# CodexploreRepo/deepfm

Hardware: AMD Instinct MI355X
Metric: train samples/sec DeepFM Criteo-shape bs4096 (higher is better)
Workload: dtype f32

## Files before the change

### deepfm_amd/_lib.py

```python

from __future__ import annotations

import ctypes as C
import os
from typing import Optional

_HERE = os.path.dirname(os.path.abspath(__file__))
LIB_PATH = os.environ.get("DFM_LIB_PATH") or os.path.join(_HERE, "lib", "libdeepfm_hip.so")

ABI_VERSION = 8

MAX_FIELDS = 64
MAX_RANKS = 64
ROWPLAN_CHUNK = 4096
SPARSE, DENSE, SEQUENCE = 0, 1, 2
COMBINER = {"mean": 0, "sum": 1, "max": 2}

c_float_p = C.c_void_p
c_int_p = C.c_void_p


class Field(C.Structure):
    _fields_ = [("kind", C.c_int32), ("dim", C.c_int32), ("vocab", C.c_int32), ("max_len", C.c_int32),
                ("combiner", C.c_int32), ("flat_offset", C.c_int32), ("stride2", C.c_int32),
# ... 98 lines not shown
    "dfm_bn_relu_dropout_backward": (_I, [_P, _P, _P, _P, _P, _L, _I, _F, _P, _I, _P, _P, _P, _P, _P]),
    "dfm_bce_workspace_bytes": (_SZ, [_L]),
    "dfm_bce_with_logits": (_I, [_P, _P, _L, _P, _P, _P, _P]),
    "dfm_gemm_workspace_bytes": (_SZ, [_I, _I, _I]),
    "dfm_gemm_f32": (_I, [_P, _L, _I, _P, _L, _I, _P, _L, _I, _I, _I, _P, _I, _P, _P]),
    "dfm_weight_grad_workspace_bytes": (_SZ, [_L, _I, _I]),
    "dfm_weight_grad_f32": (_I, [_P, _L, _P, _L, _L, _I, _I, _P, _L, _P, _I, _P, _P]),
    "dfm_attention_core_supported": (_I, [_I, _I, _I]),
    "dfm_attention_core_forward": (_I, [_P, _L, _I, _I, _I, _P, _P]),
    "dfm_attention_core_backward": (_I, [_P, _P, _L, _I, _I, _I, _P, _P]),
    "dfm_attention_qkv_core_supported": (_I, [_I, _I, _I, _I]),
    "dfm_attention_qkv_core_forward": (_I, [_P, _P, _P, _L, _I, _I, _I, _I, _P, _P]),
    "dfm_attention_qkv_core_backward": (_I, [_P, _P, _P, _P, _L, _I, _I, _I, _I, _P, _P]),
    "dfm_attention_block_supported": (_I, [_I, _I, _I, _I]),
    "dfm_attention_block_forward": (_I, [_P, _P, _P, _P, _P, _P, _P, _F, _L, _I, _I, _I, _I, _P, _P, _P, _P, _L, _P, _L,
                                         _P]),
    "dfm_attention_block_backward": (_I, [_P, _P, _P, _P, _P, _I, _L, _I, _I, _I, _I, _P, _P, _P, _L, _P, _P, _P]),
    "dfm_layernorm_workspace_bytes": (_SZ, [_L, _I]),
    "dfm_layernorm_forward": (_I, [_P, _P, _L, _I, _P, _P, _F, _P, _P, _L, _L, _P]),
    "dfm_layernorm_backward": (_I, [_P, _P, _P, _P, _L, _I, _P, _P, _P, _P, _P, _L, _L, _P]),
    "dfm_linear_bn_workspace_bytes": (_SZ, [_L, _I]),
    "dfm_linear_bn_forward": (_I, [_P, _L, _P, _P, _L, _I, _I, _P, _P, _P]),
    "dfm_bn_relu_dropout_apply": (_I, [_P, _L, _I, _P, _P, _P, _P, _P, _P, _P, _F, _F, _F, _P, _I, _P, _P]),
    "dfm_bn_bwd_workspace_bytes": (_SZ, [_L, _I]),
    "dfm_bn_backward_apply": (_I, [C.POINTER(BnBwd), _L, _I, C.POINTER(HeadTail), _P, _P]),
    "dfm_linear1_supported": (_I, [_I]),
    "dfm_linear1_forward": (_I, [_P, _L, _I, _P, _P, _P, _P]),
    "dfm_linear1_backward_splits": (_I, [_L]),
    "dfm_linear1_backward": (_I, [_P, _P, _L, _I, _P, _P, _P, _P]),
    "dfm_head_bce": (_I, [_P, _L, _I, _P, _P, _P, _P, _P, _P, _P, C.POINTER(BnBwd), _P]),
    "dfm_head_bn_bce": (_I, [_P, _P, _P, _P, _P, _F, _F, _L, _I, _P, _P, _P, _P, _P, _P, _P, C.POINTER(BnBwd), _P]),
    "dfm_linear_backward_workspace_bytes": (_SZ, [_L, _I, _I]),
    "dfm_linear_backward": (_I, [_P, _L, _I, _P, _I, _P, _P, C.POINTER(BnBwd), C.POINTER(FmBwd), _I, _P, _P]),
    "dfm_linear_backward_finish": (_I, [C.POINTER(SlabRef), _I, _P]),
    "dfm_linear_backward_splits": (_I, [_L, _I, _I]),
    "dfm_step_embedding_backward": (_I, [_P, _I, C.POINTER(_P), C.POINTER(FieldGrad), C.POINTER(C.c_int32), _I, _I, _I,
                                         _L, _P, _P, _P, _P, _P, _P, _P, _P, _I, _P, _L, _P]),
    "dfm_step_prepare_num_partials": (_L, [_I, _I, _I, _L]),
    "dfm_step_match_bytes": (_SZ, [_I, _I]),
    "dfm_step_prepare": (_I, [C.POINTER(Table), _I, _I, _I, _P, _P, _P, _P, _P, _F, _F, _P, _P, _L, _L,
                              C.POINTER(SlabRef), _I, _P, _I, _L, _P, _L, _P, _P]),
    "dfm_step_apply": (_I, [C.POINTER(Table), _I, _I, _I, _P, _P, _P, _P, _P, _P, _F, _F, _F, _F, _P, _P, _P, _P, _P,
                            _L, _I, _P]),
    "dfm_step_apply_plan": (_I, [C.POINTER(Table), _I, _I, _I, _P, _P, _P, _P, _P, _P, _F, _F, _F, _F, _P, _P, _P, _P, _P,
                                 _L, _I, _P, _L, _P, _I, _L, _P, _P, _P, _P, _P, _P]),
    "dfm_step_apply_plan_update": (_I, [_P, _P, C.POINTER(Table), _I, _I, _I, _P, _P, _P, _P, _P, _P, _F, _F, _F, _F, _P,
                                        _P, _P, _P, _P, _L, _I, _P, _L, _P, _I, _L, _P, _P, _P, _P, _P]),
    "dfm_step_apply_opt": (_I, [C.POINTER(Table), _I, _I, _I, _P, _P, _P, _P, _P, _P, C.POINTER(Optim), _P, _P, _P, _P,
                                _P, _L, _I, _P]),
    "dfm_step_apply_plan_opt": (_I, [C.POINTER(Table), _I, _I, _I, _P, _P, _P, _P, _P, _P, C.POINTER(Optim), _P, _P, _P,
                                     _P, _P, _L, _I, _P, _L, _P, _I, _L, _P, _P, _P, _P, _P, _P]),
    "dfm_step_apply_plan_opt_update": (_I, [_P, _P, C.POINTER(Table), _I, _I, _I, _P, _P, _P, _P, _P, _P,
                                            C.POINTER(Optim), _P, _P, _P, _P, _P, _L, _I, _P, _L, _P, _I, _L, _P, _P, _P,
                                            _P, _P]),
    "dfm_weight_grad_partial_blocks": (_I, [_L]),
    "dfm_weight_grad_partials_f32": (_I, [_P, _L, _P, _L, _L, _I, _I, _P, _P]),
    "dfm_weight_grad_partials_pair_f32": (_I, [_P, _L, _P, _L, _I, _I, _P, _P, _L, _P, _L, _I, _I, _P, _L, _P]),
    "dfm_layernorm_partial_blocks": (_I, [_L]),
    "dfm_partials_finish": (_I, [C.POINTER(PartialJob), _I, _P]),
    "dfm_tower_set_mode": (_I, [_I]),
    "dfm_tower_get_mode": (_I, []),
    "dfm_planes_bytes": (_SZ, [_L, _L]),
    "dfm_tower_x6_supported": (_I, [_L, _I, _I]),
    "dfm_split_planes": (_I, [C.POINTER(SplitJob), _I, _P]),
    "dfm_linear_bn_forward_x6": (_I, [_P, _L, _P, _P, _P, _L, _I, _I, _P, _P, _P]),
    "dfm_bn_relu_dropout_apply_planes": (_I, [_P, _L, _I, _P, _P, _P, _P, _P, _P, _P, _F, _F, _F, _P, _I, _P, _P, _P,
# ... 70 lines not shown
```

### deepfm_amd/csrc/gemm_core.h

```cpp
#pragma once

#include <type_traits>

#include "common.h"

namespace dfm {
namespace gemm {

typedef float f32x16 __attribute__((ext_vector_type(16)));

constexpr int BM = 64, BN = 64, BK = 32;
constexpr int LDS_STRIDE = BK + 1;
constexpr int kThreads = 512;

struct Smem {
  float a[2][BM * LDS_STRIDE];
  float b[2][BN * LDS_STRIDE];
};

struct TilePos {
  int tile, khalf;
  int wm, wn;
  int r, hf;
  __device__ __forceinline__ TilePos() {
// ... 52 lines not shown
__device__ __forceinline__ void store_slice(float* __restrict__ lds, const float4& vin, bool okv) {
  const int p = threadIdx.x;
  const float4 v = (!MASK || okv) ? vin : make_float4(0.f, 0.f, 0.f, 0.f);
  if (KC) {
    const int row = p >> 3, kq = (p & 7) * 4;
    float* d = lds + row * LDS_STRIDE + kq;
    d[0] = v.x; d[1] = v.y; d[2] = v.z; d[3] = v.w;
  } else {
    const int kk = p >> 4, rq = (p & 15) * 4;
    float* d = lds + rq * LDS_STRIDE + kk;
    d[0] = v.x; d[LDS_STRIDE] = v.y; d[2 * LDS_STRIDE] = v.z; d[3 * LDS_STRIDE] = v.w;
  }
}

template <bool KC, bool MASK, int J>
__device__ __forceinline__ void store_piece(float* __restrict__ lds, const float4& vin, bool okv) {
  const int p = threadIdx.x;
  const float e = J == 0 ? vin.x : (J == 1 ? vin.y : (J == 2 ? vin.z : vin.w));
  const float v = (!MASK || okv) ? e : 0.f;
  if (KC) lds[(p >> 3) * LDS_STRIDE + (p & 7) * 4 + J] = v;
  else lds[((p & 15) * 4 + J) * LDS_STRIDE + (p >> 4)] = v;
}

#ifndef GEMM_INTERLEAVE
#define GEMM_INTERLEAVE 1
#endif
#ifndef GEMM_INTERLEAVE_TAIL
#define GEMM_INTERLEAVE_TAIL 0
#endif
#ifndef GEMM_ABLATE
#define GEMM_ABLATE 0
#endif

constexpr int kPrefetch = 4;
constexpr int kFrag = BK / 4;

__device__ __forceinline__ void read_frags(const Smem& sm, int buf, const TilePos& pos, float (&fa)[kFrag],
                                           float (&fb)[kFrag]) {
  const float* pa = sm.a[buf] + (pos.wm + pos.r) * LDS_STRIDE + pos.hf + pos.khalf * (BK / 2);
  const float* pb = sm.b[buf] + (pos.wn + pos.r) * LDS_STRIDE + pos.hf + pos.khalf * (BK / 2);
#pragma unroll
  for (int i = 0; i < kFrag; ++i) { fa[i] = pa[2 * i]; fb[i] = pb[2 * i]; }
}

template <bool A_KC, bool B_KC, bool A_FAST, bool B_FAST, int J, bool CHECK>
__device__ __forceinline__ void pipe_step(const float* __restrict__ A, int64_t lda, const float* __restrict__ B,
                                          int64_t ldb, int M, int N, int m0, int n0, int kc, int ke, Smem& sm,
                                          const TilePos& pos, const SteadyPtr<A_KC>& spa, const SteadyPtr<B_KC>& spb,
                                          float4 (&va)[kPrefetch], float4 (&vb)[kPrefetch], bool (&oka)[kPrefetch],
                                          bool (&okb)[kPrefetch], float (&fa)[kFrag], float (&fb)[kFrag], f32x16& acc) {
  constexpr int b1 = (J + 1) & 1, b2 = J & 1, slot = (J + 2) % kPrefetch;
  constexpr bool kBareA = !CHECK && A_FAST, kBareB = !CHECK && B_FAST;
  if (CHECK && kc >= ke) return;
  float na[kFrag], nb[kFrag];
  if constexpr (GEMM_INTERLEAVE && (!CHECK || GEMM_INTERLEAVE_TAIL)) {
    const float* pa = sm.a[b1] + (pos.wm + pos.r) * LDS_STRIDE + pos.hf + pos.khalf * (BK / 2);
    const float* pb = sm.b[b1] + (pos.wn + pos.r) * LDS_STRIDE + pos.hf + pos.khalf * (BK / 2);
    static_assert(kFrag == 8, "the gap schedule below is written for 8 MFMAs per slice");
#define DFM_GAP(I, STORE)                                                                   \
    if (!(GEMM_ABLATE & 1)) acc = __builtin_amdgcn_mfma_f32_32x32x2f32(fa[I], fb[I], acc, 0, 0, 0); \
    else acc[I] += fa[I] + fb[I];                                                            \
    if (!(GEMM_ABLATE & 8)) { na[I] = pa[2 * (I)]; nb[I] = pb[2 * (I)]; } else { na[I] = fa[I]; nb[I] = fb[I]; } \
    if (!(GEMM_ABLATE & 4)) { STORE; }                                                      \
    __builtin_amdgcn_sched_barrier(0);
    __builtin_amdgcn_sched_barrier(0);
    DFM_GAP(0, (store_piece<A_KC, !kBareA, 0>(sm.a[b2], va[slot], oka[slot])))
    DFM_GAP(1, (store_piece<A_KC, !kBareA, 1>(sm.a[b2], va[slot], oka[slot])))
    DFM_GAP(2, (store_piece<A_KC, !kBareA, 2>(sm.a[b2], va[slot], oka[slot])))
    DFM_GAP(3, (store_piece<A_KC, !kBareA, 3>(sm.a[b2], va[slot], oka[slot])))
    DFM_GAP(4, (store_piece<B_KC, !kBareB, 0>(sm.b[b2], vb[slot], okb[slot])))
    DFM_GAP(5, (store_piece<B_KC, !kBareB, 1>(sm.b[b2], vb[slot], okb[slot])))
    DFM_GAP(6, (store_piece<B_KC, !kBareB, 2>(sm.b[b2], vb[slot], okb[slot])))
    DFM_GAP(7, (store_piece<B_KC, !kBareB, 3>(sm.b[b2], vb[slot], okb[slot])))
#undef DFM_GAP
    if (!(GEMM_ABLATE & 2)) {
    if (kBareA) { va[slot] = spa.load(kc + (kPrefetch + 2) * BK); oka[slot] = true; }
    else load_slice<A_KC, A_FAST>(A, lda, m0, M, kc + (kPrefetch + 2) * BK, ke, va[slot], oka[slot]);
    if (kBareB) { vb[slot] = spb.load(kc + (kPrefetch + 2) * BK); okb[slot] = true; }
    else load_slice<B_KC, B_FAST>(B, ldb, n0, N, kc + (kPrefetch + 2) * BK, ke, vb[slot], okb[slot]);
    }
    __builtin_amdgcn_sched_barrier(0);
  } else {
#pragma unroll
  for (int i = 0; i < kFrag; ++i) na[i] = nb[i] = 0.f;
  if (!CHECK || kc + BK < ke) read_frags(sm, b1, pos, na, nb);
  if (!CHECK || kc + 2 * BK < ke) {
    store_slice<A_KC, !kBareA>(sm.a[b2], va[slot], oka[slot]);
    store_slice<B_KC, !kBareB>(sm.b[b2], vb[slot], okb[slot]);
  }
  if (!CHECK || kc + (kPrefetch + 2) * BK < ke) {
    if (kBareA) { va[slot] = spa.load(kc + (kPrefetch + 2) * BK); oka[slot] = true; }
    else load_slice<A_KC, A_FAST>(A, lda, m0, M, kc + (kPrefetch + 2) * BK, ke, va[slot], oka[slot]);
    if (kBareB) { vb[slot] = spb.load(kc + (kPrefetch + 2) * BK); okb[slot] = true; }
    else load_slice<B_KC, B_FAST>(B, ldb, n0, N, kc + (kPrefetch + 2) * BK, ke, vb[slot], okb[slot]);
  }
  __builtin_amdgcn_sched_barrier(0);
#pragma unroll
  for (int i = 0; i < kFrag; ++i) acc = __builtin_amdgcn_mfma_f32_32x32x2f32(fa[i], fb[i], acc, 0, 0, 0);
  __builtin_amdgcn_sched_barrier(0);
  }
  if (!(GEMM_ABLATE & 16) || CHECK) __syncthreads();
#pragma unroll
  for (int i = 0; i < kFrag; ++i) { fa[i] = na[i]; fb[i] = nb[i]; }
}

template <bool A_KC, bool B_KC, bool A_FAST, bool B_FAST>
__device__ __forceinline__ void mainloop(const float* __restrict__ A, int64_t lda, const float* __restrict__ B,
                                         int64_t ldb, int M, int N, int m0, int n0, int kb, int ke, Smem& sm,
                                         const TilePos& pos, f32x16& acc) {
  static_assert(kPrefetch == 4, "the slot schedule below is written out for 4 slices in flight");
  const int lane = lane_id();
  float4 va[kPrefetch], vb[kPrefetch];
  bool oka[kPrefetch], okb[kPrefetch];
#pragma unroll
  for (int j = 0; j < kPrefetch; ++j) {
    oka[j] = okb[j] = false;
    va[j] = vb[j] = make_float4(0.f, 0.f, 0.f, 0.f);
    if (kb + j * BK < ke) {
      load_slice<A_KC, A_FAST>(A, lda, m0, M, kb + j * BK, ke, va[j], oka[j]);
      load_slice<B_KC, B_FAST>(B, ldb, n0, N, kb + j * BK, ke, vb[j], okb[j]);
    }
  }
  store_slice<A_KC>(sm.a[0], va[0], oka[0]);
  store_slice<B_KC>(sm.b[0], vb[0], okb[0]);
  store_slice<A_KC>(sm.a[1], va[1], oka[1]);
  store_slice<B_KC>(sm.b[1], vb[1], okb[1]);
#pragma unroll
  for (int j = 0; j < 2; ++j) {
    if (kb + (kPrefetch + j) * BK < ke) {
      load_slice<A_KC, A_FAST>(A, lda, m0, M, kb + (kPrefetch + j) * BK, ke, va[j], oka[j]);
      load_slice<B_KC, B_FAST>(B, ldb, n0, N, kb + (kPrefetch + j) * BK, ke, vb[j], okb[j]);
    }
  }
  __syncthreads();
  float fa[kFrag], fb[kFrag];
  read_frags(sm, 0, pos, fa, fb);
  __syncthreads();
  const SteadyPtr<A_KC> spa(A, lda, m0, M);
  const SteadyPtr<B_KC> spb(B, ldb, n0, N);
#define DFM_PIPE(J, CHECK)                                                                                       \
  pipe_step<A_KC, B_KC, A_FAST, B_FAST, J, CHECK>(A, lda, B, ldb, M, N, m0, n0, k0 + (J) * BK, ke, sm, pos, spa, \
                                                  spb, va, vb, oka, okb, fa, fb, acc)
  int k0 = kb;
  __builtin_amdgcn_s_waitcnt(0x0F70);
  for (; k0 + (kPrefetch + 6) * BK <= ke; k0 += kPrefetch * BK) {
    DFM_PIPE(0, false); DFM_PIPE(1, false); DFM_PIPE(2, false); DFM_PIPE(3, false);
  }
  for (; k0 < ke; k0 += kPrefetch * BK) {
    DFM_PIPE(0, true); DFM_PIPE(1, true); DFM_PIPE(2, true); DFM_PIPE(3, true);
  }
#undef DFM_PIPE
  float* park = &sm.a[0][0];
  if (pos.khalf == 1) {
#pragma unroll
    for (int reg = 0; reg < 16; ++reg) park[(pos.tile * 16 + reg) * 64 + lane] = acc[reg];
  }
  __syncthreads();
  if (pos.khalf == 0) {
#pragma unroll
    for (int reg = 0; reg < 16; ++reg) acc[reg] += park[(pos.tile * 16 + reg) * 64 + lane];
  }
  __syncthreads();
}

typedef __bf16 bf16x8 __attribute__((ext_vector_type(8)));
typedef __bf16 bf16x2 __attribute__((ext_vector_type(2)));
constexpr int BKX = 64;
constexpr int kPlane = 4 * 2 * 64 * 8;
struct SmemX3 {
  __bf16 a[2][2][kPlane];
  __bf16 b[2][2][kPlane];
};
static_assert(sizeof(SmemX3) == 64 * 1024, "two operands x two buffers x (hi, lo) x 8 KB");

template <bool KC>
struct PieceX3 {
  const float* ptr;
  int64_t kstep;
  int k_off;
  int lds0;
  __device__ __forceinline__ PieceX3(const float* base, int64_t ld, int r0, int rows) {
    const int p = threadIdx.x;
    if (KC) {
      const int r = r0 + (p >> 3), k8 = p & 7;
      const int rc = r < rows ? r : rows - 1;
      ptr = base + static_cast<int64_t>(rc) * ld;
      kstep = 1; k_off = 8 * k8;
      lds0 = (((k8 >> 1) * 2 + (k8 & 1)) * 64 + (p >> 3)) * 8;
    } else {
      const int kq = p >> 4, r = r0 + (p & 15) * 4;
      const int rc = r < rows ? r : rows - 4;
      ptr = base + rc;
      kstep = ld; k_off = 2 * kq;
      const int k = 2 * kq;
      lds0 = ((((k >> 4) * 2 + ((k >> 3) & 1)) * 64 + (p & 15) * 4) * 8) + (k & 7);
// ... 126 lines not shown
```

### deepfm_amd/csrc/tower.hip

```cpp
#include "dropout.h"
#include "gemm_core.h"
#include "gemm_x6.h"

using namespace dfm;
using namespace dfm::gemm;

namespace {


struct BnBwd {
  const float* z;
  const float* mean_rstd;
  const float* gamma;
  const float* beta;
  float* dy;
  float* g_gamma;
  float* g_beta;
  const int64_t* seed;
  float* partial;
  uint32_t thresh;
  float inv_keep;
  int salt;
};

// ... 510 lines not shown
  float* g[kMaxSlabRefs];
  int elems4[kMaxSlabRefs];
  int splits[kMaxSlabRefs];
  int first_block[kMaxSlabRefs + 1];
  int count;
};
__global__ __launch_bounds__(256) void slab_reduce_kernel(SlabRefs refs) {
  int e = 0;
  while (e + 1 < refs.count && static_cast<int>(blockIdx.x) >= refs.first_block[e + 1]) ++e;
  const int i4 = (blockIdx.x - refs.first_block[e]) * 256 + threadIdx.x;
  if (i4 >= refs.elems4[e]) return;
  const float* sl = refs.slabs[e] + static_cast<int64_t>(i4) * 4;
  const int64_t stride = static_cast<int64_t>(refs.elems4[e]) * 4;
  const int splits = refs.splits[e];
  float4 acc = make_float4(0.f, 0.f, 0.f, 0.f);
  int q = 0;
  for (; q + 8 <= splits; q += 8) {
    float4 t[8];
#pragma unroll
    for (int u = 0; u < 8; ++u) t[u] = ld4(sl + (q + u) * stride);
#pragma unroll
    for (int u = 0; u < 8; ++u) { acc.x += t[u].x; acc.y += t[u].y; acc.z += t[u].z; acc.w += t[u].w; }
  }
  for (; q < splits; ++q) {
    const float4 t = ld4(sl + q * stride);
    acc.x += t.x; acc.y += t.y; acc.z += t.z; acc.w += t.w;
  }
  float* g = refs.g[e] + static_cast<int64_t>(i4) * 4;
  const float4 old = ld4(g);
  st4(g, make_float4(old.x + acc.x, old.y + acc.y, old.z + acc.z, old.w + acc.w));
}

namespace {
inline int tiles(int n, int t) { return (n + t - 1) / t; }
inline size_t align256(size_t b) { return (b + 255) / 256 * 256; }
inline bool aligned16(const void* p) { return (reinterpret_cast<uintptr_t>(p) & 15) == 0; }

inline size_t tile_partial_bytes(int64_t m, int n) { return align256(sizeof(float) * 2 * static_cast<size_t>((m + 31) / 32) * n); }
inline size_t head_partial_bytes(int64_t m, int k) {
  return align256(sizeof(float) * static_cast<size_t>((m + kHeadRows - 1) / kHeadRows) * (3 * static_cast<size_t>(k) + 4));
}

int dw_splits(int n_out, int k_in, int64_t m) {
  constexpr int64_t kRound = 512;
  const int64_t t = static_cast<int64_t>(tiles(n_out, BM)) * tiles(k_in, BN);
  const int64_t dx = ((m + BM - 1) / BM) * tiles(k_in, BN);
  const int64_t max_s = m / (4 * BK) > 0 ? m / (4 * BK) : 1;
  int64_t room = (dx / kRound + 1) * kRound - dx;
  int64_t s = room / t;
  if (s < 4 && max_s >= 4) s = (room + kRound) / t;
  if (s > max_s) s = max_s;
  return s < 1 ? 1 : static_cast<int>(s);
}

bool fill_bn(const dfm_bn_bwd* h, BnBwd* d) {
  if (!h->z || !h->mean_rstd || !h->gamma || !h->beta || !h->dy || !h->g_gamma || !h->g_beta || !h->workspace)
    return false;
  if (!(h->p_drop >= 0.f && h->p_drop < 1.f) || (h->p_drop > 0.f && !h->seed)) return false;
  d->z = h->z; d->mean_rstd = h->mean_rstd; d->gamma = h->gamma; d->beta = h->beta;
  d->dy = h->dy; d->g_gamma = h->g_gamma; d->g_beta = h->g_beta;
  d->seed = h->seed;
  d->partial = static_cast<float*>(h->workspace);
  d->thresh = dropout_thresh(h->p_drop);
  d->inv_keep = 1.f / (1.f - h->p_drop);
  d->salt = h->salt;
  return true;
// ... 329 lines not shown
  if (bn_below && (parts & 2)) DFM_REQUIRE(fill_bn(bn_below, &dbn), "incomplete dfm_bn_bwd");
  FmBwd dfm_ = {};
  if (fm && (parts & 2)) {
    DFM_REQUIRE(fm->g_fm || fm->addend, "dfm_fm_bwd: neither an FM gradient nor an addend");
    DFM_REQUIRE(!fm->g_fm || (fm->fm_sum && fm->e && fm->dim > 0 && K % fm->dim == 0), "incomplete dfm_fm_bwd");
    dfm_.g_fm = fm->g_fm; dfm_.fm_sum = fm->fm_sum; dfm_.e = fm->e; dfm_.addend = fm->addend;
    dfm_.dim = fm->dim > 0 ? fm->dim : 1;
  }
  int splits, k_per_split;
  dw_split_plan(N, K, M, &splits, &k_per_split);
  const int dw_tn = tiles(K, BN), dw_t = tiles(N, BM) * dw_tn;
  const int dx_tn = tiles(K, BN), dx_t = tiles(M, BM) * dx_tn;
  float* slabs = static_cast<float*>(d_workspace);
  const bool fast = operand_fast(d_dz, N, false, N, M) && operand_fast(d_x, K, false, K, M) &&
                    operand_fast(d_dz, N, true, M, N) && operand_fast(d_w, K, false, K, N);
  const int dw_blocks = (parts & 1) ? dw_t * splits : 0;
  const dim3 grid(static_cast<unsigned>(dw_blocks + ((parts & 2) ? dx_t : 0)));
#define DFM_LBWD(F, E)                                                                                            \
  hipLaunchKernelGGL((linear_bwd_kernel<F, E>), grid, dim3(kThreads), 0, as_stream(stream), d_dz, d_x, d_w,        \
                     d_g_x, M, N, K, dw_tn, dw_t, splits, dw_blocks, k_per_split, slabs, dx_tn, dbn, dfm_)
  const int epi = bn_below ? 1 : (fm ? 2 : 0);
  if (g_tower_mode == 1 && fast && N % 8 == 0 && M % 2 == 0 && k_per_split % 2 == 0) {
#define DFM_LBWD3(E)                                                                                              \
  hipLaunchKernelGGL((linear_bwd_kernel<true, E, true>), grid, dim3(kThreads), 0, as_stream(stream), d_dz, d_x,    \
                     d_w, d_g_x, M, N, K, dw_tn, dw_t, splits, dw_blocks, k_per_split, slabs, dx_tn, dbn, dfm_)
    if (epi == 0) DFM_LBWD3(0); else if (epi == 1) DFM_LBWD3(1); else DFM_LBWD3(2);
#undef DFM_LBWD3
  } else if (fast) {
    if (epi == 0) DFM_LBWD(true, 0); else if (epi == 1) DFM_LBWD(true, 1); else DFM_LBWD(true, 2);
  } else {
    if (epi == 0) DFM_LBWD(false, 0); else if (epi == 1) DFM_LBWD(false, 1); else DFM_LBWD(false, 2);
  }
#undef DFM_LBWD
  DFM_LAUNCH_CHECK();
  return DFM_OK;
}

namespace {
constexpr int kMaxSplitJobs = 8;
struct SplitJobs {
  const float* src[kMaxSplitJobs];
  int rows[kMaxSplitJobs], cols[kMaxSplitJobs], tiles_c[kMaxSplitJobs];
  Planes f[kMaxSplitJobs], s[kMaxSplitJobs];
  int first_block[kMaxSplitJobs + 1];
  int count;
};
}

__global__ __launch_bounds__(kApThreads) void split_planes_kernel(SplitJobs jobs) {
  __shared__ __attribute__((aligned(16))) float tile[kTileRows * kTileStride];
  int e = 0;
  while (e + 1 < jobs.count && static_cast<int>(blockIdx.x) >= jobs.first_block[e + 1]) ++e;
  const int lb = blockIdx.x - jobs.first_block[e];
  const int R = jobs.rows[e], C = jobs.cols[e];
  const int r0 = (lb / jobs.tiles_c[e]) * kTileRows, c0 = (lb % jobs.tiles_c[e]) * kTileCols;
  const int cl = threadIdx.x & 15, rl = threadIdx.x >> 4;
  const float* src = jobs.src[e];
#pragma unroll
  for (int i = 0; i < kTileRows / kApRowLanes; ++i) {
    const int m = r0 + rl + i * kApRowLanes, c = c0 + cl * 4;
    float4 v = make_float4(0.f, 0.f, 0.f, 0.f);
    if (m < R && c < C) v = ld4(src + static_cast<int64_t>(m) * C + c);
    st4(&tile[(rl + i * kApRowLanes) * kTileStride + cl * 4], v);
  }
  __syncthreads();
  emit_planes_from_tile(tile, r0, c0, R, C, jobs.f[e], jobs.s[e]);
// ... 235 lines not shown
```

### deepfm_amd/training/fused_step.py

```python

from __future__ import annotations

import ctypes as C
import os
from typing import List, Optional

import torch

from deepfm_amd import _lib
from deepfm_amd.training.rowsparse import RowSparseOptimizer
from deepfm_amd.training.step import RowSparseTrainStep


def _zeros_bytes(nbytes: int, device) -> torch.Tensor:
    return torch.zeros(max((nbytes + 3) // 4, 1), dtype=torch.int32, device=device)


def _tower_ok(model) -> bool:
    if not model.training:
        return False
    dnn = getattr(model, "dnn", None)
    if dnn is None or not getattr(dnn, "_fusable", False):
        return False
    widths = [dnn.mlp[4 * i].out_features for i in range(dnn._n_layers)]
# ... 32 lines not shown
        self.lin, self.bn, self.drop_p = [], [], []
        self.z, self.a, self.stats, self.dy = [], [], [], []
        self.ws_fwd, self.ws_bn, self.ws_lin = [], [], []
        for i in range(self.L):
            lin, bn, _, drop = (dnn.mlp[4 * i + j] for j in range(4))
            n, k = lin.out_features, lin.in_features
            self.lin.append(lin); self.bn.append(bn); self.drop_p.append(float(drop.p))
            self.z.append(torch.empty(B, n, **f32))
            self.a.append(torch.empty(B, n, **f32))
            self.dy.append(torch.empty(B, n, **f32))
            self.stats.append(torch.empty(2, n, **f32))
            self.ws_fwd.append(_zeros_bytes(lib.dfm_linear_bn_workspace_bytes(B, n), dev))
            self.ws_bn.append(_zeros_bytes(lib.dfm_bn_bwd_workspace_bytes(B, n), dev))
            self.ws_lin.append(_zeros_bytes(lib.dfm_linear_backward_workspace_bytes(B, n, k), dev))
        self.tower_mode = int(lib.dfm_tower_get_mode())
        self.x6 = self.tower_mode == 2 and all(
            lib.dfm_tower_x6_supported(B, l.out_features, l.in_features) for l in self.lin)
        if self.x6:
            def planes(rows, contraction):
                return _zeros_bytes(lib.dfm_planes_bytes(rows, contraction), dev)
            self.w_f = [planes(l.out_features, l.in_features) for l in self.lin]
            self.w_s = [planes(l.in_features, l.out_features) for l in self.lin]
            self.a_f = [planes(B, l.out_features) for l in self.lin[:-1]]
            self.a_s = [planes(l.out_features, B) for l in self.lin[:-1]]
            self.dz_f = [planes(B, l.out_features) for l in self.lin]
            self.dz_s = [planes(l.out_features, B) for l in self.lin]
            self.ws_lin = [_zeros_bytes(lib.dfm_linear_backward_x6_workspace_bytes(B, l.out_features, l.in_features), dev)
                           for l in self.lin]
            self._split_jobs = (_lib.SplitJob * self.L)()
            for i, l in enumerate(self.lin):
                j = self._split_jobs[i]
                j.src, j.rows, j.cols = l.weight.data_ptr(), l.out_features, l.in_features
                j.planes_f, j.planes_s = self.w_f[i].data_ptr(), self.w_s[i].data_ptr()
        self.seed = torch.randint(1, 2 ** 40, (1,), dtype=torch.int64, device=dev)
        if torch.distributed.is_available() and torch.distributed.is_initialized():
            self.seed += 7919 * torch.distributed.get_rank()
        optimizer.seed_tick = self.seed
        self.rowplan_side_stream = os.environ.get("DFM_ROWPLAN_SIDE_STREAM") == "1"
        self.head = getattr(model, self.head_name)
        for p in list(dnn.parameters()) + list(self.head.parameters()):
            if p.grad is None or not p.grad.is_contiguous():
                raise RuntimeError("fused steps need RowSparseAdam's flat gradient views on every dense parameter")

    def _tower_input(self) -> torch.Tensor:
        return self.fe.view(self.B, -1)

    def _tower_input_grad(self) -> torch.Tensor:
        return self.g_fe

    def _finish_embedding_grad(self) -> None:
        """After the tower's backward: whatever is still missing in ``g_fe`` (default: nothing)."""

    def _interaction_forward(self) -> Optional[torch.Tensor]:
        raise NotImplementedError

    def _interaction_backward(self) -> Optional[_lib.FmBwd]:
        raise NotImplementedError

    def _bn_ctx(self, i: int) -> _lib.BnBwd:
        bn = self.bn[i]
        c = _lib.BnBwd()
        c.z, c.mean_rstd = self.z[i].data_ptr(), self.stats[i].data_ptr()
        c.gamma, c.beta = bn.weight.data_ptr(), bn.bias.data_ptr()
        c.dy = self.dy[i].data_ptr()
        c.g_gamma, c.g_beta = bn.weight.grad.data_ptr(), bn.bias.grad.data_ptr()
        c.seed = self.seed.data_ptr()
# ... 42 lines not shown
                    self.logits.data_ptr(), self.g_logits.data_ptr(), C.byref(ctx), st))
                break
            if x6:
                _lib.check(lib.dfm_bn_relu_dropout_apply_planes(
                    self.z[i].data_ptr(), B, n, self.ws_fwd[i].data_ptr(), bn.weight.data_ptr(), bn.bias.data_ptr(),
                    *stats, self.drop_p[i], self.seed.data_ptr(), i, None, self.a_f[i].data_ptr(),
                    self.a_s[i].data_ptr(), st))
            else:
                _lib.check(lib.dfm_bn_relu_dropout_apply(
                    self.z[i].data_ptr(), B, n, self.ws_fwd[i].data_ptr(), bn.weight.data_ptr(), bn.bias.data_ptr(),
                    *stats, self.drop_p[i], self.seed.data_ptr(), i, self.a[i].data_ptr(), st))
            x = self.a[i]
        tail = _lib.HeadTail()
        tail.g_w = head.weight.grad.data_ptr()
        tail.g_b = head.bias.grad.data_ptr() if head.bias is not None else None
        tail.loss = self.loss.data_ptr()
        tail.g_b2 = self._second_logit_bias_grad()
        fmb = self._interaction_backward()
        for i in range(self.L - 1, -1, -1):
            lin = self.lin[i]
            n, k = lin.out_features, lin.in_features
            if x6:
                _lib.check(lib.dfm_bn_backward_apply_planes(
                    C.byref(ctx), B, n, C.byref(tail) if i == self.L - 1 else None, None, self.dz_f[i].data_ptr(),
                    self.dz_s[i].data_ptr(), st))
                if i > 0:
                    ctx = self._bn_ctx(i - 1)
                _lib.check(lib.dfm_linear_backward_x6(
                    self.dz_f[i].data_ptr(), self.dz_s[i].data_ptr(), B, n, self.x0.data_ptr() if i == 0 else None,
                    self.a_s[i - 1].data_ptr() if i > 0 else None, k, self.w_s[i].data_ptr(),
                    self.g_x0.data_ptr() if i == 0 else None, C.byref(ctx) if i > 0 else None,
                    C.byref(fmb) if (i == 0 and fmb is not None) else None, self.ws_lin[i].data_ptr(), st))
                continue
            _lib.check(lib.dfm_bn_backward_apply(C.byref(ctx), B, n, C.byref(tail) if i == self.L - 1 else None,
                                                 self.dy[i].data_ptr(), st))
            xin = self.a[i - 1] if i > 0 else self.x0
            if i > 0:
                ctx = self._bn_ctx(i - 1)
                _lib.check(lib.dfm_linear_backward(
                    self.dy[i].data_ptr(), B, n, xin.data_ptr(), k, lin.weight.data_ptr(), None, C.byref(ctx),
                    None, 3, self.ws_lin[i].data_ptr(), st))
            else:
                _lib.check(lib.dfm_linear_backward(
                    self.dy[i].data_ptr(), B, n, xin.data_ptr(), k, lin.weight.data_ptr(), self.g_x0.data_ptr(),
                    None, C.byref(fmb) if fmb is not None else None, 3, self.ws_lin[i].data_ptr(), st))
        self._finish_embedding_grad()
        extra = self._extra_slab_refs()
        n_refs = self.L + (1 if self._dense_parts else 0) + len(extra)
        refs = (_lib.SlabRef * n_refs)()
        for j, (ws_ptr, g_ptr, elems, splits) in enumerate(extra):
            r = refs[n_refs - len(extra) + j]
            r.workspace, r.g_w = ws_ptr, g_ptr
            r.batch, r.out_features, r.in_features, r.splits = 1, 1, elems, splits
        for i in range(self.L):
            r, lin = refs[i], self.lin[i]
            r.workspace, r.g_w = self.ws_lin[i].data_ptr(), lin.weight.grad.data_ptr()
            r.batch, r.out_features, r.in_features = B, lin.out_features, lin.in_features
            if x6:
                r.splits = lib.dfm_linear_backward_x6_splits(B, lin.out_features, lin.in_features)
        if self._dense_parts:
            r = refs[self.L]
            r.workspace, r.g_w = self._dense_partial.data_ptr(), self.opt.flat_grad.data_ptr()
            r.batch, r.out_features, r.in_features, r.splits = 1, 1, self.opt.n_l2, self._dense_parts
        if self.slabs_travel:
            self._slab_refs = (refs, n_refs)
        elif not self.opt.split:
# ... 250 lines not shown
```

### include/deepfm_hip.h

```cpp
#ifndef DEEPFM_HIP_H
#define DEEPFM_HIP_H

#include <stddef.h>
#include <stdint.h>

#ifdef __cplusplus
extern "C" {
#endif

#define DFM_ABI_VERSION 8
#define DFM_MAX_FIELDS 64
#define DFM_MAX_RANKS 64
#define DFM_ROWPLAN_CHUNK 4096

enum dfm_status { DFM_OK = 0, DFM_ERR_INVALID = 1, DFM_ERR_HIP = 2, DFM_ERR_UNSUPPORTED = 3 };
enum dfm_field_kind { DFM_SPARSE = 0, DFM_DENSE = 1, DFM_SEQUENCE = 2 };
enum dfm_combiner { DFM_MEAN = 0, DFM_SUM = 1, DFM_MAX = 2 };

typedef void* dfm_stream_t;

int dfm_abi_version(void);
const char* dfm_last_error(void);
int dfm_device_info(int* cu_count, int* wave_size, char* arch, int arch_len);
int dfm_debug_empty_launch(dfm_stream_t stream);
// ... 230 lines not shown

typedef struct dfm_head_tail {
  float* g_w;
  float* g_b;
  float* loss;
  float* g_b2;
} dfm_head_tail;

size_t dfm_linear_bn_workspace_bytes(int64_t batch, int features);
int dfm_linear_bn_forward(const float* d_x, int64_t ldx, const float* d_w, const float* d_bias,
                          int64_t batch, int out_features, int in_features, float* d_z,
                          void* d_workspace, dfm_stream_t stream);
int dfm_bn_relu_dropout_apply(const float* d_z, int64_t batch, int features, const void* d_workspace,
                              const float* d_gamma, const float* d_beta, float* d_mean_rstd,
                              float* d_running_mean, float* d_running_var, int64_t* d_num_batches,
                              float momentum, float eps, float p_drop, const int64_t* d_seed, int salt,
                              float* d_out, dfm_stream_t stream);
size_t dfm_bn_bwd_workspace_bytes(int64_t batch, int features);
int dfm_head_bce(const float* d_a, int64_t batch, int features, const float* d_w, const float* d_b,
                 const float* d_first_order, const float* d_fm, const float* d_labels, float* d_logits,
                 float* d_g_logits, const dfm_bn_bwd* bn, dfm_stream_t stream);
int dfm_head_bn_bce(const void* d_fwd_workspace, float* d_mean_rstd, float* d_running_mean, float* d_running_var,
                    int64_t* d_num_batches, float momentum, float eps, int64_t batch, int features,
                    const float* d_w, const float* d_b, const float* d_first_order, const float* d_fm,
                    const float* d_labels, float* d_logits, float* d_g_logits, const dfm_bn_bwd* bn,
                    dfm_stream_t stream);
int dfm_bn_backward_apply(const dfm_bn_bwd* bn, int64_t batch, int features, const dfm_head_tail* head,
                          float* d_dz, dfm_stream_t stream);
size_t dfm_linear_backward_workspace_bytes(int64_t batch, int out_features, int in_features);
int dfm_linear_backward(const float* d_dz, int64_t batch, int out_features, const float* d_x,
                        int in_features, const float* d_w, float* d_g_x,
                        const dfm_bn_bwd* bn_below, const dfm_fm_bwd* fm, int parts, void* d_workspace,
                        dfm_stream_t stream);
int dfm_linear1_supported(int features);
int dfm_linear1_forward(const float* d_x, int64_t batch, int features, const float* d_w, const float* d_b,
                        float* d_out, dfm_stream_t stream);
int dfm_linear1_backward_splits(int64_t batch);
int dfm_linear1_backward(const float* d_g, const float* d_x, int64_t batch, int features, const float* d_w,
                         float* d_g_x, void* d_workspace, dfm_stream_t stream);
typedef struct dfm_slab_ref {
  const void* workspace;
  float* g_w;
  int64_t batch;
  int32_t out_features;
  int32_t in_features;
  int32_t splits;
  int32_t reserved;
} dfm_slab_ref;
int dfm_linear_backward_finish(const dfm_slab_ref* refs, int count, dfm_stream_t stream);
int dfm_tower_set_mode(int mode);
int dfm_tower_get_mode(void);

size_t dfm_planes_bytes(int64_t rows, int64_t contraction);
int dfm_tower_x6_supported(int64_t batch, int out_features, int in_features);
typedef struct {
  const float* src;
  int64_t rows, cols;
  void* planes_f;
  void* planes_s;
} dfm_split_job;
int dfm_split_planes(const dfm_split_job* jobs, int count, dfm_stream_t stream);
int dfm_linear_bn_forward_x6(const float* d_x, int64_t ldx, const void* d_x_planes_f, const void* d_w_planes_f,
                             const float* d_bias, int64_t batch, int out_features, int in_features, float* d_z,
                             void* d_workspace, dfm_stream_t stream);
int dfm_bn_relu_dropout_apply_planes(const float* d_z, int64_t batch, int features, const void* d_workspace,
                                     const float* d_gamma, const float* d_beta, float* d_mean_rstd,
// ... 124 lines not shown
```

Measured before the change: 20.00 million.

## Fold BN backward apply into the tower linear backward GEMM operand load

Adds a fused kernel that reduces the BN partial sums per block, then applies the batchnorm backward transform to the dy operand as it is staged into LDS inside the GEMM mainloop, for both the dW and dX tiles. This removes the separate bn_backward_apply launch and the write and re-read of the transformed dz tensor for narrow tower layers. In exchange every block redundantly reduces the column partials, each A-slice load also fetches z and LDS stats, and register pressure in the pipelined loop rises. It is enabled by default for non-first layers with at most 64 outputs.

```diff
diff --git a/deepfm_amd/_lib.py b/deepfm_amd/_lib.py
--- a/deepfm_amd/_lib.py
+++ b/deepfm_amd/_lib.py
@@ -154,6 +154,9 @@
     "dfm_head_bn_bce": (_I, [_P, _P, _P, _P, _P, _F, _F, _L, _I, _P, _P, _P, _P, _P, _P, _P, C.POINTER(BnBwd), _P]),
     "dfm_linear_backward_workspace_bytes": (_SZ, [_L, _I, _I]),
     "dfm_linear_backward": (_I, [_P, _L, _I, _P, _I, _P, _P, C.POINTER(BnBwd), C.POINTER(FmBwd), _I, _P, _P]),
+    "dfm_tower_fold_supported": (_I, [_L, _I, _I]),
+    "dfm_linear_backward_fold": (_I, [C.POINTER(BnBwd), C.POINTER(HeadTail), _L, _I, _P, _I, _P, _P, C.POINTER(BnBwd),
+                                      C.POINTER(FmBwd), _P, _P]),
     "dfm_linear_backward_finish": (_I, [C.POINTER(SlabRef), _I, _P]),
     "dfm_linear_backward_splits": (_I, [_L, _I, _I]),
     "dfm_step_embedding_backward": (_I, [_P, _I, C.POINTER(_P), C.POINTER(FieldGrad), C.POINTER(C.c_int32), _I, _I, _I,
diff --git a/deepfm_amd/csrc/gemm_core.h b/deepfm_amd/csrc/gemm_core.h
--- a/deepfm_amd/csrc/gemm_core.h
+++ b/deepfm_amd/csrc/gemm_core.h
@@ -108,6 +108,11 @@
 #define GEMM_ABLATE 0
 #endif
 
+struct NoXform {
+  __device__ __forceinline__ void prefetch(int, int, int) {}
+  __device__ __forceinline__ void apply(float4&, int, int, int) {}
+};
+
 constexpr int kPrefetch = 4;
 constexpr int kFrag = BK / 4;
 
@@ -119,12 +124,13 @@
   for (int i = 0; i < kFrag; ++i) { fa[i] = pa[2 * i]; fb[i] = pb[2 * i]; }
 }
 
-template <bool A_KC, bool B_KC, bool A_FAST, bool B_FAST, int J, bool CHECK>
+template <bool A_KC, bool B_KC, bool A_FAST, bool B_FAST, int J, bool CHECK, class AX>
 __device__ __forceinline__ void pipe_step(const float* __restrict__ A, int64_t lda, const float* __restrict__ B,
                                           int64_t ldb, int M, int N, int m0, int n0, int kc, int ke, Smem& sm,
                                           const TilePos& pos, const SteadyPtr<A_KC>& spa, const SteadyPtr<B_KC>& spb,
                                           float4 (&va)[kPrefetch], float4 (&vb)[kPrefetch], bool (&oka)[kPrefetch],
-                                          bool (&okb)[kPrefetch], float (&fa)[kFrag], float (&fb)[kFrag], f32x16& acc) {
+                                          bool (&okb)[kPrefetch], float (&fa)[kFrag], float (&fb)[kFrag], f32x16& acc,
+                                          AX& ax) {
   constexpr int b1 = (J + 1) & 1, b2 = J & 1, slot = (J + 2) % kPrefetch;
   constexpr bool kBareA = !CHECK && A_FAST, kBareB = !CHECK && B_FAST;
   if (CHECK && kc >= ke) return;
@@ -140,7 +146,7 @@
     if (!(GEMM_ABLATE & 4)) { STORE; }                                                      \
     __builtin_amdgcn_sched_barrier(0);
     __builtin_amdgcn_sched_barrier(0);
-    DFM_GAP(0, (store_piece<A_KC, !kBareA, 0>(sm.a[b2], va[slot], oka[slot])))
+    DFM_GAP(0, (ax.apply(va[slot], slot, kc + 2 * BK, ke), store_piece<A_KC, !kBareA, 0>(sm.a[b2], va[slot], oka[slot])))
     DFM_GAP(1, (store_piece<A_KC, !kBareA, 1>(sm.a[b2], va[slot], oka[slot])))
     DFM_GAP(2, (store_piece<A_KC, !kBareA, 2>(sm.a[b2], va[slot], oka[slot])))
     DFM_GAP(3, (store_piece<A_KC, !kBareA, 3>(sm.a[b2], va[slot], oka[slot])))
@@ -152,6 +158,7 @@
     if (!(GEMM_ABLATE & 2)) {
     if (kBareA) { va[slot] = spa.load(kc + (kPrefetch + 2) * BK); oka[slot] = true; }
     else load_slice<A_KC, A_FAST>(A, lda, m0, M, kc + (kPrefetch + 2) * BK, ke, va[slot], oka[slot]);
+    ax.prefetch(slot, kc + (kPrefetch + 2) * BK, ke);
     if (kBareB) { vb[slot] = spb.load(kc + (kPrefetch + 2) * BK); okb[slot] = true; }
     else load_slice<B_KC, B_FAST>(B, ldb, n0, N, kc + (kPrefetch + 2) * BK, ke, vb[slot], okb[slot]);
     }
@@ -161,12 +168,14 @@
   for (int i = 0; i < kFrag; ++i) na[i] = nb[i] = 0.f;
   if (!CHECK || kc + BK < ke) read_frags(sm, b1, pos, na, nb);
   if (!CHECK || kc + 2 * BK < ke) {
+    ax.apply(va[slot], slot, kc + 2 * BK, ke);
     store_slice<A_KC, !kBareA>(sm.a[b2], va[slot], oka[slot]);
     store_slice<B_KC, !kBareB>(sm.b[b2], vb[slot], okb[slot]);
   }
   if (!CHECK || kc + (kPrefetch + 2) * BK < ke) {
     if (kBareA) { va[slot] = spa.load(kc + (kPrefetch + 2) * BK); oka[slot] = true; }
     else load_slice<A_KC, A_FAST>(A, lda, m0, M, kc + (kPrefetch + 2) * BK, ke, va[slot], oka[slot]);
+    ax.prefetch(slot, kc + (kPrefetch + 2) * BK, ke);
     if (kBareB) { vb[slot] = spb.load(kc + (kPrefetch + 2) * BK); okb[slot] = true; }
     else load_slice<B_KC, B_FAST>(B, ldb, n0, N, kc + (kPrefetch + 2) * BK, ke, vb[slot], okb[slot]);
   }
@@ -180,10 +189,10 @@
   for (int i = 0; i < kFrag; ++i) { fa[i] = na[i]; fb[i] = nb[i]; }
 }
 
-template <bool A_KC, bool B_KC, bool A_FAST, bool B_FAST>
-__device__ __forceinline__ void mainloop(const float* __restrict__ A, int64_t lda, const float* __restrict__ B,
-                                         int64_t ldb, int M, int N, int m0, int n0, int kb, int ke, Smem& sm,
-                                         const TilePos& pos, f32x16& acc) {
+template <bool A_KC, bool B_KC, bool A_FAST, bool B_FAST, class AX>
+__device__ __forceinline__ void mainloop_ax(const float* __restrict__ A, int64_t lda, const float* __restrict__ B,
+                                            int64_t ldb, int M, int N, int m0, int n0, int kb, int ke, Smem& sm,
+                                            const TilePos& pos, f32x16& acc, AX& ax) {
   static_assert(kPrefetch == 4, "the slot schedule below is written out for 4 slices in flight");
   const int lane = lane_id();
   float4 va[kPrefetch], vb[kPrefetch];
@@ -194,17 +203,21 @@
     va[j] = vb[j] = make_float4(0.f, 0.f, 0.f, 0.f);
     if (kb + j * BK < ke) {
       load_slice<A_KC, A_FAST>(A, lda, m0, M, kb + j * BK, ke, va[j], oka[j]);
+      ax.prefetch(j, kb + j * BK, ke);
       load_slice<B_KC, B_FAST>(B, ldb, n0, N, kb + j * BK, ke, vb[j], okb[j]);
     }
   }
+  ax.apply(va[0], 0, kb, ke);
   store_slice<A_KC>(sm.a[0], va[0], oka[0]);
   store_slice<B_KC>(sm.b[0], vb[0], okb[0]);
+  ax.apply(va[1], 1, kb + BK, ke);
   store_slice<A_KC>(sm.a[1], va[1], oka[1]);
   store_slice<B_KC>(sm.b[1], vb[1], okb[1]);
 #pragma unroll
   for (int j = 0; j < 2; ++j) {
     if (kb + (kPrefetch + j) * BK < ke) {
       load_slice<A_KC, A_FAST>(A, lda, m0, M, kb + (kPrefetch + j) * BK, ke, va[j], oka[j]);
+      ax.prefetch(j, kb + (kPrefetch + j) * BK, ke);
       load_slice<B_KC, B_FAST>(B, ldb, n0, N, kb + (kPrefetch + j) * BK, ke, vb[j], okb[j]);
     }
   }
@@ -216,7 +229,7 @@
   const SteadyPtr<B_KC> spb(B, ldb, n0, N);
 #define DFM_PIPE(J, CHECK)                                                                                       \
   pipe_step<A_KC, B_KC, A_FAST, B_FAST, J, CHECK>(A, lda, B, ldb, M, N, m0, n0, k0 + (J) * BK, ke, sm, pos, spa, \
-                                                  spb, va, vb, oka, okb, fa, fb, acc)
+                                                  spb, va, vb, oka, okb, fa, fb, acc, ax)
   int k0 = kb;
   __builtin_amdgcn_s_waitcnt(0x0F70);
   for (; k0 + (kPrefetch + 6) * BK <= ke; k0 += kPrefetch * BK) {
@@ -237,6 +250,14 @@
     for (int reg = 0; reg < 16; ++reg) acc[reg] += park[(pos.tile * 16 + reg) * 64 + lane];
   }
   __syncthreads();
+}
+
+template <bool A_KC, bool B_KC, bool A_FAST, bool B_FAST>
+__device__ __forceinline__ void mainloop(const float* __restrict__ A, int64_t lda, const float* __restrict__ B,
+                                         int64_t ldb, int M, int N, int m0, int n0, int kb, int ke, Smem& sm,
+                                         const TilePos& pos, f32x16& acc) {
+  NoXform nx;
+  mainloop_ax<A_KC, B_KC, A_FAST, B_FAST>(A, lda, B, ldb, M, N, m0, n0, kb, ke, sm, pos, acc, nx);
 }
 
 typedef __bf16 bf16x8 __attribute__((ext_vector_type(8)));
diff --git a/deepfm_amd/csrc/tower.hip b/deepfm_amd/csrc/tower.hip
--- a/deepfm_amd/csrc/tower.hip
+++ b/deepfm_amd/csrc/tower.hip
@@ -566,6 +566,163 @@
 }
 
 namespace {
+constexpr int kFoldMaxK = 512;
+constexpr int kFoldCols = 2 * kApCols;
+
+__device__ __forceinline__ void half_row_lane_totals(float4& a, float4& b, float (*red)[kApRowLanes][kApCols], int cl,
+                                                     int rl) {
+  st4(&red[0][rl][cl * 4], a);
+  st4(&red[1][rl][cl * 4], b);
+  __syncthreads();
+  float4 ta = make_float4(0.f, 0.f, 0.f, 0.f), tb = ta;
+#pragma unroll
+  for (int i = 0; i < kApRowLanes; ++i) {
+    const float4 x = ld4(&red[0][i][cl * 4]), y = ld4(&red[1][i][cl * 4]);
+    ta.x += x.x; ta.y += x.y; ta.z += x.z; ta.w += x.w;
+    tb.x += y.x; tb.y += y.y; tb.z += y.z; tb.w += y.w;
+  }
+  __syncthreads();
+  a = ta; b = tb;
+}
+
+static_assert(sizeof(float) * 2 * 2 * kApRowLanes * kApCols <= sizeof(Smem::a), "merge scratch must fit in sm.a");
+__device__ __forceinline__ float (*fold_red(Smem& sm, int half))[kApRowLanes][kApCols] {
+  return reinterpret_cast<float (*)[kApRowLanes][kApCols]>(&sm.a[0][0]) + 2 * half;
+}
+
+template <bool KC>
+struct BwdFoldA {
+  const float* z;
+  const float* s_mu; const float* s_rs; const float* s_ga; const float* s_m1; const float* s_m2;
+  int rows, ld, r0;
+  float4 vz[kPrefetch];
+  __device__ __forceinline__ void piece(int k0, int ke, int64_t& off, int& f) const {
+    const int p = threadIdx.x;
+    int r, k;
+    if (KC) { r = r0 + (p >> 3); k = k0 + (p & 7) * 4; }
+    else    { k = k0 + (p >> 4); r = r0 + (p & 15) * 4; }
+    const int rc = KC ? (r < rows ? r : rows - 1) : (r < rows ? r : rows - 4);
+    const int kc = k < ke ? k : 0;
+    off = KC ? static_cast<int64_t>(rc) * ld + kc : static_cast<int64_t>(kc) * ld + rc;
+    f = KC ? kc : rc;
+  }
+  __device__ __forceinline__ void prefetch(int slot, int k0, int ke) {
+    int64_t off; int f;
+    piece(k0, ke, off, f);
+    vz[slot] = ld4(z + off);
+  }
+  __device__ __forceinline__ void apply(float4& v, int slot, int k0, int ke) {
+    int64_t off; int f;
+    piece(k0, ke, off, f);
+    const float4 zv = vz[slot];
+    const float4 muv = ld4(s_mu + f), rsv = ld4(s_rs + f), gav = ld4(s_ga + f), m1v = ld4(s_m1 + f), m2v = ld4(s_m2 + f);
+    const float mu[4] = {muv.x, muv.y, muv.z, muv.w}, rs[4] = {rsv.x, rsv.y, rsv.z, rsv.w};
+    const float ga[4] = {gav.x, gav.y, gav.z, gav.w};
+    const float m1[4] = {m1v.x, m1v.y, m1v.z, m1v.w}, m2[4] = {m2v.x, m2v.y, m2v.z, m2v.w};
+    const float dd[4] = {v.x, v.y, v.z, v.w}, zz[4] = {zv.x, zv.y, zv.z, zv.w};
+    float o[4];
+#pragma unroll
+    for (int u = 0; u < 4; ++u) o[u] = ga[u] * rs[u] * (dd[u] - m1[u] - (zz[u] - mu[u]) * rs[u] * m2[u]);
+    v = make_float4(o[0], o[1], o[2], o[3]);
+  }
+};
+
+template <int EPI>
+__global__ __launch_bounds__(kThreads) void linear_bwd_fold_kernel(
+    BnBwd bn, int T, int stride, int off1, HeadTail head, const float* __restrict__ x, const float* __restrict__ w,
+    float* __restrict__ g_x, int M, int N, int K, int dw_tiles_n, int dw_tiles, int dw_blocks, int k_per_split,
+    float* __restrict__ slabs, int dx_tiles_n, BnBwd below, FmBwd fmb) {
+  __shared__ Smem sm;
+  __shared__ __attribute__((aligned(16))) float s_col[5][kFoldMaxK];
+  const TilePos pos;
+  const int wg = blockIdx.x;
+  const int bid = wg < dw_blocks ? xcd_logical_index(wg, dw_blocks)
+                                 : dw_blocks + xcd_logical_index_from(wg - dw_blocks, static_cast<int>(gridDim.x) - dw_blocks, dw_blocks);
+  const bool is_dw = bid < dw_blocks;
+  const int tile = bid % (dw_tiles > 0 ? dw_tiles : 1);
+  const int f0 = is_dw ? (tile / dw_tiles_n) * BM : 0;
+  const int f1 = is_dw ? (f0 + BM < N ? f0 + BM : N) : N;
+  const bool lead = bid == dw_blocks;
+  {
+    const int half = threadIdx.x >> 8, cl = threadIdx.x & 15, rl = (threadIdx.x >> 4) & 15;
+    float (*red)[kApRowLanes][kApCols] = fold_red(sm, half);
+    const float invM = 1.f / static_cast<float>(M);
+    for (int c0 = f0; c0 < f1; c0 += kFoldCols) {
+      const int c = c0 + half * kApCols + cl * 4;
+      const bool okc = c < f1;
+      const int cc = okc ? c : 0;
+      float4 s1 = make_float4(0.f, 0.f, 0.f, 0.f), s2 = s1;
+#pragma unroll 8
+      for (int t = rl; t < T; t += kApRowLanes) {
+        const float4 a = ld4(bn.partial + static_cast<int64_t>(t) * stride + cc);
+        const float4 b = ld4(bn.partial + static_cast<int64_t>(t) * stride + off1 + cc);
+        s1.x += a.x; s1.y += a.y; s1.z += a.z; s1.w += a.w;
+        s2.x += b.x; s2.y += b.y; s2.z += b.z; s2.w += b.w;
+      }
+      half_row_lane_totals(s1, s2, red, cl, rl);
+      if (lead) {
+        if (rl == 0 && okc) {
+          const float4 gb = ld4(bn.g_beta + c), gg = ld4(bn.g_gamma + c);
+          st4(bn.g_beta + c, make_float4(gb.x + s1.x, gb.y + s1.y, gb.z + s1.z, gb.w + s1.w));
+          st4(bn.g_gamma + c, make_float4(gg.x + s2.x, gg.y + s2.y, gg.z + s2.z, gg.w + s2.w));
+        }
+        if (head.enabled) {
+          float4 s3 = make_float4(0.f, 0.f, 0.f, 0.f), s4 = s3;
+#pragma unroll 4
+          for (int t = rl; t < T; t += kApRowLanes) {
+            const float4 a = ld4(bn.partial + static_cast<int64_t>(t) * stride + 2 * off1 + cc);
+            s3.x += a.x; s3.y += a.y; s3.z += a.z; s3.w += a.w;
+            if (cl == 0) {
+              s4.x += bn.partial[static_cast<int64_t>(t) * stride + 3 * off1];
+              s4.y += bn.partial[static_cast<int64_t>(t) * stride + 3 * off1 + 1];
+            }
+          }
+          half_row_lane_totals(s3, s4, red, cl, rl);
+          if (rl == 0 && okc) {
+            const float4 gw = ld4(head.g_w + c);
+            st4(head.g_w + c, make_float4(gw.x + s3.x, gw.y + s3.y, gw.z + s3.z, gw.w + s3.w));
+          }
+          if (c0 == 0 && half == 0 && cl == 0 && rl == 0) {
+            head.loss[0] = s4.x / static_cast<float>(M);
+            if (head.g_b) head.g_b[0] += s4.y;
+            if (head.g_b2) head.g_b2[0] += s4.y;
+          }
+        }
+      }
+      if (rl == 0 && okc) {
+        st4(&s_col[0][c], ld4(bn.mean_rstd + c));
+        st4(&s_col[1][c], ld4(bn.mean_rstd + N + c));
+        st4(&s_col[2][c], ld4(bn.gamma + c));
+        st4(&s_col[3][c], make_float4(s1.x * invM, s1.y * invM, s1.z * invM, s1.w * invM));
+        st4(&s_col[4][c], make_float4(s2.x * invM, s2.y * invM, s2.z * invM, s2.w * invM));
+      }
+    }
+    __syncthreads();
+  }
+  f32x16 acc = {};
+  if (is_dw) {
+    const int sp = bid / dw_tiles;
+    const int m0 = f0, n0 = (tile % dw_tiles_n) * BN;
+    const int kb = sp * k_per_split;
+    const int ke = kb + k_per_split < M ? kb + k_per_split : M;
+    BwdFoldA<false> ax;
+    ax.z = bn.z; ax.s_mu = s_col[0]; ax.s_rs = s_col[1]; ax.s_ga = s_col[2]; ax.s_m1 = s_col[3]; ax.s_m2 = s_col[4];
+    ax.rows = N; ax.ld = N; ax.r0 = m0;
+    mainloop_ax<false, false, true, true>(bn.dy, N, x, K, N, K, m0, n0, kb, ke, sm, pos, acc, ax);
+    dw_tile_store(acc, pos, m0, n0, N, K, slabs + static_cast<int64_t>(sp) * N * K);
+    return;
+  }
+  const int t = bid - dw_blocks;
+  const int m0 = (t / dx_tiles_n) * BM, n0 = (t % dx_tiles_n) * BN;
+  BwdFoldA<true> ax;
+  ax.z = bn.z; ax.s_mu = s_col[0]; ax.s_rs = s_col[1]; ax.s_ga = s_col[2]; ax.s_m1 = s_col[3]; ax.s_m2 = s_col[4];
+  ax.rows = M; ax.ld = N; ax.r0 = m0;
+  mainloop_ax<true, false, true, true>(bn.dy, N, w, K, M, K, m0, n0, 0, N, sm, pos, acc, ax);
+  dx_tile_epilogue<EPI>(acc, pos, m0, n0, M, K, g_x, below, fmb);
+}
+}
+
+namespace {
 inline int tiles(int n, int t) { return (n + t - 1) / t; }
 inline size_t align256(size_t b) { return (b + 255) / 256 * 256; }
 inline bool aligned16(const void* p) { return (reinterpret_cast<uintptr_t>(p) & 15) == 0; }
@@ -961,6 +1118,59 @@
     if (epi == 0) DFM_LBWD(false, 0); else if (epi == 1) DFM_LBWD(false, 1); else DFM_LBWD(false, 2);
   }
 #undef DFM_LBWD
+  DFM_LAUNCH_CHECK();
+  return DFM_OK;
+}
+
+extern "C" int dfm_tower_fold_supported(int64_t batch, int out_features, int in_features) {
+  return batch > 0 && batch < (1 << 30) && out_features > 0 && out_features % 4 == 0 && out_features <= kFoldMaxK &&
+         in_features > 0 && in_features % 4 == 0;
+}
+
+extern "C" int dfm_linear_backward_fold(const dfm_bn_bwd* bn, const dfm_head_tail* head, int64_t batch,
+                                        int out_features, const float* d_x, int in_features, const float* d_w,
+                                        float* d_g_x, const dfm_bn_bwd* bn_below, const dfm_fm_bwd* fm,
+                                        void* d_workspace, dfm_stream_t stream) {
+  DFM_REQUIRE(bn && d_x && d_w && d_workspace, "null argument");
+  DFM_REQUIRE(dfm_tower_fold_supported(batch, out_features, in_features),
+              "fold: features %% 4 == 0, at most %d", kFoldMaxK);
+  DFM_REQUIRE((bn_below != nullptr) != (fm != nullptr), "exactly one of bn_below / fm");
+  DFM_REQUIRE(bn_below || d_g_x, "d_g_x is required with fm");
+  const int M = static_cast<int>(batch), N = out_features, K = in_features;
+  BnBwd d = {};
+  DFM_REQUIRE(fill_bn(bn, &d), "incomplete dfm_bn_bwd");
+  DFM_REQUIRE(aligned16(d.dy) && aligned16(d.z) && aligned16(d.mean_rstd) && aligned16(d.gamma) &&
+                  aligned16(d.partial) && aligned16(d.g_gamma) && aligned16(d.g_beta) && aligned16(d_x) &&
+                  aligned16(d_w), "pointers must be 16-byte aligned");
+  HeadTail ht = {};
+  int T = (M + 31) / 32, stride = 2 * N, off1 = N;
+  if (head) {
+    DFM_REQUIRE(head->g_w && head->loss && aligned16(head->g_w), "incomplete dfm_head_tail");
+    ht.g_w = head->g_w; ht.g_b = head->g_b; ht.loss = head->loss; ht.g_b2 = head->g_b2; ht.enabled = 1;
+    T = (M + kHeadRows - 1) / kHeadRows;
+    stride = 3 * N + 4;
+  }
+  BnBwd below = {};
+  if (bn_below) DFM_REQUIRE(fill_bn(bn_below, &below), "incomplete dfm_bn_bwd");
+  FmBwd fmb = {};
+  if (fm) {
+    DFM_REQUIRE(fm->g_fm || fm->addend, "dfm_fm_bwd: neither an FM gradient nor an addend");
+    DFM_REQUIRE(!fm->g_fm || (fm->fm_sum && fm->e && fm->dim > 0 && K % fm->dim == 0), "incomplete dfm_fm_bwd");
+    fmb.g_fm = fm->g_fm; fmb.fm_sum = fm->fm_sum; fmb.e = fm->e; fmb.addend = fm->addend;
+    fmb.dim = fm->dim > 0 ? fm->dim : 1;
+  }
+  int splits, k_per_split;
+  dw_split_plan(N, K, M, &splits, &k_per_split);
+  const int dw_tn = tiles(K, BN), dw_t = tiles(N, BM) * dw_tn;
+  const int dx_tn = tiles(K, BN), dx_t = tiles(M, BM) * dx_tn;
+  const int dw_blocks = dw_t * splits;
+  const dim3 grid(static_cast<unsigned>(dw_blocks + dx_t));
+  float* slabs = static_cast<float*>(d_workspace);
+#define DFM_LBWDF(E)                                                                                              \
+  hipLaunchKernelGGL((linear_bwd_fold_kernel<E>), grid, dim3(kThreads), 0, as_stream(stream), d, T, stride, off1,  \
+                     ht, d_x, d_w, d_g_x, M, N, K, dw_tn, dw_t, dw_blocks, k_per_split, slabs, dx_tn, below, fmb)
+  if (bn_below) DFM_LBWDF(1); else DFM_LBWDF(2);
+#undef DFM_LBWDF
   DFM_LAUNCH_CHECK();
   return DFM_OK;
 }
diff --git a/deepfm_amd/training/fused_step.py b/deepfm_amd/training/fused_step.py
--- a/deepfm_amd/training/fused_step.py
+++ b/deepfm_amd/training/fused_step.py
@@ -88,6 +88,14 @@
                 j = self._split_jobs[i]
                 j.src, j.rows, j.cols = l.weight.data_ptr(), l.out_features, l.in_features
                 j.planes_f, j.planes_s = self.w_f[i].data_ptr(), self.w_s[i].data_ptr()
+        fold_env = os.environ.get("DFM_TOWER_FOLD", "1")
+        if fold_env not in ("0", "1", "all"):
+            raise ValueError(f"DFM_TOWER_FOLD={fold_env!r}: expected 0, 1 or all")
+        self.fold_layers = frozenset(
+            i for i in range(self.L)
+            if self.tower_mode == 0 and fold_env != "0"
+            and (fold_env == "all" or (i > 0 and self.lin[i].out_features <= 64))
+            and lib.dfm_tower_fold_supported(B, self.lin[i].out_features, self.lin[i].in_features))
         self.seed = torch.randint(1, 2 ** 40, (1,), dtype=torch.int64, device=dev)
         if torch.distributed.is_available() and torch.distributed.is_initialized():
             self.seed += 7919 * torch.distributed.get_rank()
@@ -196,6 +204,15 @@
                     self.g_x0.data_ptr() if i == 0 else None, C.byref(ctx) if i > 0 else None,
                     C.byref(fmb) if (i == 0 and fmb is not None) else None, self.ws_lin[i].data_ptr(), st))
                 continue
+            if i in self.fold_layers and (i > 0 or fmb is not None):
+                below = self._bn_ctx(i - 1) if i > 0 else None
+                _lib.check(lib.dfm_linear_backward_fold(
+                    C.byref(ctx), C.byref(tail) if i == self.L - 1 else None, B, n,
+                    (self.a[i - 1] if i > 0 else self.x0).data_ptr(), k, lin.weight.data_ptr(),
+                    None if i > 0 else self.g_x0.data_ptr(), C.byref(below) if i > 0 else None,
+                    C.byref(fmb) if i == 0 else None, self.ws_lin[i].data_ptr(), st))
+                ctx = below
+                continue
             _lib.check(lib.dfm_bn_backward_apply(C.byref(ctx), B, n, C.byref(tail) if i == self.L - 1 else None,
                                                  self.dy[i].data_ptr(), st))
             xin = self.a[i - 1] if i > 0 else self.x0
diff --git a/include/deepfm_hip.h b/include/deepfm_hip.h
--- a/include/deepfm_hip.h
+++ b/include/deepfm_hip.h
@@ -286,6 +286,11 @@
                         int in_features, const float* d_w, float* d_g_x,
                         const dfm_bn_bwd* bn_below, const dfm_fm_bwd* fm, int parts, void* d_workspace,
                         dfm_stream_t stream);
+int dfm_tower_fold_supported(int64_t batch, int out_features, int in_features);
+int dfm_linear_backward_fold(const dfm_bn_bwd* bn, const dfm_head_tail* head, int64_t batch, int out_features,
+                             const float* d_x, int in_features, const float* d_w, float* d_g_x,
+                             const dfm_bn_bwd* bn_below, const dfm_fm_bwd* fm, void* d_workspace,
+                             dfm_stream_t stream);
 int dfm_linear1_supported(int features);
 int dfm_linear1_forward(const float* d_x, int64_t batch, int features, const float* d_w, const float* d_b,
                         float* d_out, dfm_stream_t stream);
```

After: 20.07 million, median of 6. About the same (+0.4%).
